# colmap/pycolmap

Hardware: AMD Instinct MI355X
Metric: descriptor-pair distances/sec (exhaustive SIFT match: dot + top-2 + ratio + cross-check) (higher is better)
Workload: dtype u8 descriptors, int8 MFMA / int32 accumulate; 1 GPU; 500 images x 4096 descriptors, exhaustive match + ratio test + cross-check (BASELINE.json configs[1] at N=1); pairs_total=124750, pairs_per_rank=124750, kernel=auto, matches_rank0=1865611

## Files before the change

### pycolmap_amd/csrc/match_mfma.hip

```cpp
#include <cstdlib>

#include "amc_internal.h"
#include "scan_accept.h"

namespace amc {

typedef int i32x4 __attribute__((ext_vector_type(4)));
typedef __attribute__((address_space(1))) const void gvoid_t;
typedef __attribute__((address_space(3))) void lvoid_t;

constexpr int kBN = 256;
constexpr int kYS = kBN / 32;
constexpr int kUR = 128;
constexpr int kSPB = kUR / 32;
constexpr int kUPC = kBN / kUR;
constexpr int kChunkBytes = kBN * kDim;
constexpr int kW = kSegsPerItem;
constexpr int kXT = kSegRows / 16;
constexpr int kKeyShift = 7, kKeyCarried = 127;

constexpr int kNB = 3;
constexpr int kOffRs = 0;
constexpr int kOffQ = kOffRs + kNB * kBN * 4;
constexpr int kOffB = kOffQ + 16;
constexpr int kLdsBytes = kOffB + kNB * kChunkBytes;
static_assert(kBN == kRowPad, "a chunk is the row padding unit");
static_assert(kUR == 128 && kSPB == 4, "a lane quarter's rows of a block are one 32-row tile; the loop body is one block");
static_assert(kRowPad % kSegRows == 0 && kSegRows % 32 == 0, "segments tile the padded rows");
static_assert(kLdsBytes <= 160 * 1024, "LDS of one CU");
static_assert(sizeof(SegDesc) == 64, "a descriptor is 16 dwords: one per lane of a quarter wave");

enum : int { kDXprep = 0, kDXrs = 2, kDOut = 4, kDList = 6, kDYprep = 8, kDYrs = 10, kDCnt = 12, kDAccword = 13,
             kDYrows = 14 };

__device__ __forceinline__ void mfma_first(i32x4& d, const i32x4& a, const i32x4& b, const i32x4& c) {
    asm volatile("v_mfma_i32_16x16x64_i8 %0, %1, %2, %3" : "=&v"(d) : "v"(a), "v"(b), "v"(c));
}
__device__ __forceinline__ void mfma_acc(i32x4& d, const i32x4& a, const i32x4& b) {
    asm volatile("v_mfma_i32_16x16x64_i8 %0, %1, %2, %0" : "+v"(d) : "v"(a), "v"(b));
}

struct YFrag {
    i32x4 f[2][2];
    i32x4 ci[2];
};

#ifdef AMC_SCAN_STAMPS
constexpr int kStampMaxWG = 1024;
__device__ uint32_t g_scan_stamps[2 * kStampMaxWG * kSegsPerItem * 8];
#define AMC_STAMP() ((uint32_t)__builtin_amdgcn_s_memtime())
#endif

__device__ __noinline__ __attribute__((used)) void copy_part(const uint4* __restrict__ src, uint4* __restrict__ dst,
                                                             unsigned long long b, unsigned long long e, int tid,
                                                             int nthreads) {
    __builtin_assume(tid >= 0 && tid < 1024 && nthreads >= 256 && nthreads <= 512);
    unsigned long long i = b + (unsigned long long)tid;
    const unsigned long long st = (unsigned long long)nthreads;
    for (; i + 3 * st < e; i += 4 * st) {
        const uint4 v0 = src[i], v1 = src[i + st], v2 = src[i + 2 * st], v3 = src[i + 3 * st];
        dst[i] = v0; dst[i + st] = v1; dst[i + 2 * st] = v2; dst[i + 3 * st] = v3;
    }
    for (; i < e; i += st) dst[i] = src[i];
}

template <int MODE>
__global__ __launch_bounds__(64 * kW) void match_mfma_kernel(const SegDesc* __restrict__ segs,
                                                             const uint32_t* __restrict__ nitems_p,
                                                             uint32_t* __restrict__ queue_head,
                                                             uint32_t* __restrict__ accmask,
                                                             const ScanAccept* __restrict__ accept,
                                                             CopyJob job, uint32_t* __restrict__ copy_head) {
    static_assert((kChunkBytes / 1024) % kW == 0 && kYS % (kChunkBytes / 1024 / kW) == 0, "a chunk splits into 1 KiB DMA pieces per wave, dealt evenly over its steps");
    __shared__ __attribute__((aligned(16))) char smem[kLdsBytes];

    const int tid = threadIdx.x;
    const int lane = tid & 63;
    const int wid = __builtin_amdgcn_readfirstlane(tid >> 6);
    const int l15 = lane & 15, lq = lane >> 4;
    volatile uint32_t* s_q = reinterpret_cast<volatile uint32_t*>(smem + kOffQ);
    if constexpr (MODE == 0) {
        if (job.parts) {
            __shared__ uint32_t s_part;
            if (tid == 0) s_part = atomicAdd(copy_head, 1u);
            __syncthreads();
            const uint32_t part = s_part;
            if (part < job.parts)
                copy_part(static_cast<const uint4*>(job.src), static_cast<uint4*>(job.dst), job.n16 * part / job.parts,
                          job.n16 * (part + 1) / job.parts, tid, 64 * kW);
        }
    }
    const uint32_t nitems = *nitems_p;
    const ScanAccept sa = *accept;

    auto load_desc = [&](uint32_t q) -> int {
        int v = 0;
        if (q < nitems && lane < 16) v = reinterpret_cast<const int*>(segs + (size_t)q * kSegsPerItem + wid)[lane];
        return v;
    };
    auto dword = [&](int dv, int f) -> int { return __builtin_amdgcn_readlane(dv, f); };
    auto dptr = [&](int dv, int f) -> const char* {
        const uint64_t lo = (uint32_t)__builtin_amdgcn_readlane(dv, f);
        const uint64_t hi = (uint32_t)__builtin_amdgcn_readlane(dv, f + 1);
        return reinterpret_cast<const char*>(lo | (hi << 32));
    };

    constexpr int kPW = kChunkBytes / 1024 / kW;
    auto stage_piece = [&](const char* yprep, int c, int buf, int ps) __attribute__((always_inline)) {
        const int piece = ps * kW + wid;
        __builtin_amdgcn_global_load_lds((gvoid_t*)(yprep + (size_t)c * kChunkBytes + piece * 1024 + lane * 16),
                                         (lvoid_t*)(smem + kOffB + buf * kChunkBytes + piece * 1024), 16, 0, 0);
    };
    auto stage_rs = [&](const char* yrs, int c, int buf) __attribute__((always_inline)) {
        if (wid == 0)
            __builtin_amdgcn_global_load_lds((gvoid_t*)(yrs + (size_t)c * kBN * 4 + lane * 16),
                                             (lvoid_t*)(smem + kOffRs + buf * kBN * 4), 16, 0, 0);
    };
    auto stage = [&](const char* yprep, const char* yrs, int c, int buf) __attribute__((always_inline)) {
#pragma unroll
        for (int ps = 0; ps < kPW; ++ps) stage_piece(yprep, c, buf, ps);
        stage_rs(yrs, c, buf);
    };

    const int yrow_lane = (kUR / 4) * (l15 >> 2) + (l15 & 3);
    const int ysw_lane = arena_swizzle(yrow_lane);
    const int yoff0 = kOffB + yrow_lane * kDim + ((lq ^ ysw_lane) * 16);
    const int yoff1 = kOffB + yrow_lane * kDim + (((4 + lq) ^ ysw_lane) * 16);
    const int coff = kOffRs + (kUR / 4) * lq * 4;
    auto load_y_part = [&](YFrag& y, int buf, int ys, int part) __attribute__((always_inline)) {
        const int ub = (ys / kSPB) * kUR, sp = ys % kSPB;
        if (part < 2) {
            const int so = buf * kBN * 4 + (ub + 8 * sp) * 4;
            y.ci[part] = *reinterpret_cast<const i32x4*>(smem + (coff + so) + 16 * part);
        } else {
            const int tt = (part - 2) >> 1, s = (part - 2) & 1;
            const int so = buf * kChunkBytes + (ub + 8 * sp) * kDim;
            y.f[tt][s] = *reinterpret_cast<const i32x4*>(smem + ((s ? yoff1 : yoff0) + so) + tt * 4 * kDim);
        }
    };
    auto load_y = [&](YFrag& y, int buf, int ys) __attribute__((always_inline)) {
#pragma unroll
        for (int part = 0; part < 6; ++part) load_y_part(y, buf, ys, part);
    };

    i32x4 xf[kXT][2];
    int best[kXT], sec[kXT], btile[kXT], xterm[kXT], part[kXT];
    auto load_x = [&](int dv) __attribute__((always_inline)) {
        const int cnt = dword(dv, kDCnt);
        const char* xprep = dptr(dv, kDXprep);
        const int* xrs = reinterpret_cast<const int*>(dptr(dv, kDXrs));
#pragma unroll
        for (int xt = 0; xt < kXT; ++xt) {
            const int kl = xt * 16 + l15;
            int row;
            if (MODE == 0) {
                row = kl;
            } else {
                const uint32_t* list = reinterpret_cast<const uint32_t*>(dptr(dv, kDList));
                row = cnt > 0 ? (int)list[min(kl, cnt - 1)] : 0;
            }
            const char* rp = xprep + (size_t)row * kDim;
            const int sw = arena_swizzle(row);
#pragma unroll
            for (int s = 0; s < 2; ++s) xf[xt][s] = *reinterpret_cast<const i32x4*>(rp + (((4 * s + lq) ^ sw) * 16));
            xterm[xt] = xrs[row] - (1 << 21);
            best[xt] = ((-xterm[xt]) << kKeyShift) | kKeyCarried;
            sec[xt] = best[xt];
            btile[xt] = -1;
        }
    };

#ifdef AMC_SCAN_STAMPS
    uint32_t st_a = 0, st_first = 0, st_end = 0, st_sum[5] = {0, 0, 0, 0, 0};
    bool st_prev = false, st_prev_active = false;
    uint32_t* const st_slot = g_scan_stamps + ((size_t)(MODE * kStampMaxWG + min((int)blockIdx.x, kStampMaxWG - 1)) * kW + wid) * 8;
#endif
    if (tid == 0) *s_q = atomicAdd(queue_head, 1u);
    __syncthreads();
    uint32_t q = *s_q;
    int dv = load_desc(q);
    if (q < nitems) {
        stage(dptr(dv, kDYprep), dptr(dv, kDYrs), 0, 0);
        if (dword(dv, kDYrows) > kBN) stage(dptr(dv, kDYprep), dptr(dv, kDYrs), 1, 1);
        if (dword(dv, kDCnt) > 0) load_x(dv);
    }
    __syncthreads();

    while (q < nitems) {
        const char* yprep = dptr(dv, kDYprep);
        const char* yrs = dptr(dv, kDYrs);
        const int yrows_item = dword(dv, kDYrows);
        const int nchunks = (yrows_item + kBN - 1) / kBN;
        const int last_steps = (((yrows_item - (nchunks - 1) * kBN) + 31) / 32 + kSPB - 1) & ~(kSPB - 1);
        const bool active = dword(dv, kDCnt) > 0;
        if (tid == 0) *s_q = atomicAdd(queue_head, 1u);

        i32x4 acc[2][2];
        auto insert = [&](int xt, int code) __attribute__((always_inline)) {
            asm volatile(
                "v_lshl_or_b32 %2, %2, 7, %3\n\t"
                "v_med3_i32 %1, %0, %1, %2\n\t"
                "v_max_i32 %0, %0, %2"
                : "+v"(best[xt]), "+v"(sec[xt]), "+v"(part[xt])
                : "s"(code));
        };
        auto flush = [&](int sb) __attribute__((always_inline)) {
#pragma unroll
            for (int xt = 0; xt < kXT; ++xt) {
                const int c = best[xt] & 127;
                btile[xt] = c != kKeyCarried ? sb * 64 + (126 - c) : btile[xt];
                best[xt] |= kKeyCarried;
            }
        };
        auto phase = [&](i32x4 (&an)[2], const YFrag& y, int xtn, const i32x4 (&ac)[2], int xtc, int sp, int gb)
                         __attribute__((always_inline)) {
            mfma_first(an[0], y.f[0][0], xf[xtn][0], y.ci[0]);
            mfma_first(an[1], y.f[1][0], xf[xtn][0], y.ci[1]);
            __builtin_amdgcn_sched_barrier(0);
            if (xtc == 0 ? sp == 0 : sp == kSPB - 1) {
                insert((xtc + kXT - 1) % kXT, 126 - ((xtc == 0 ? gb - 1 : gb) & 63));
                if (xtc == 0 && gb != 0 && (gb & 63) == 0) flush((gb >> 6) - 1);
                __builtin_amdgcn_sched_barrier(0);
            }
            mfma_acc(an[0], y.f[0][1], xf[xtn][1]);
            mfma_acc(an[1], y.f[1][1], xf[xtn][1]);
            __builtin_amdgcn_sched_barrier(0);
            int t0, t1;
            if (sp == 0)
                asm volatile(
                    "v_max3_i32 %0, %3, %4, %5\n\t"
                    "v_max3_i32 %1, %6, %7, %8\n\t"
                    "v_max3_i32 %0, %0, %9, %10\n\t"
                    "v_max_i32 %2, %0, %1"
                    : "=&v"(t0), "=&v"(t1), "=&v"(part[xtc])
                    : "v"(ac[0][0]), "v"(ac[0][1]), "v"(ac[0][2]), "v"(ac[0][3]), "v"(ac[1][0]), "v"(ac[1][1]),
                      "v"(ac[1][2]), "v"(ac[1][3]));
            else
                asm volatile(
                    "v_max3_i32 %0, %3, %4, %5\n\t"
                    "v_max3_i32 %1, %6, %7, %8\n\t"
                    "v_max3_i32 %0, %0, %9, %10\n\t"
                    "v_max3_i32 %2, %0, %1, %2"
                    : "=&v"(t0), "=&v"(t1), "+v"(part[xtc])
                    : "v"(ac[0][0]), "v"(ac[0][1]), "v"(ac[0][2]), "v"(ac[0][3]), "v"(ac[1][0]), "v"(ac[1][1]),
                      "v"(ac[1][2]), "v"(ac[1][3]));
            __builtin_amdgcn_sched_barrier(0);
        };

        YFrag y0, y1;
        asm volatile("s_waitcnt vmcnt(0)" ::: "memory");
        __syncthreads();
        const uint32_t qn = *s_q;
        const int dvn = load_desc(qn);
#ifdef AMC_SCAN_STAMPS
        {
            const uint32_t now = AMC_STAMP();
            if (st_prev) {
                st_sum[0] += st_a;
                st_sum[1] += now - st_end;
                st_sum[2] += now - st_first;
                st_sum[3] += 1;
                st_sum[4] += st_prev_active ? 1 : 0;
                if (lane == 0) {
#pragma unroll
                    for (int k = 0; k < 5; ++k) st_slot[k] = st_sum[k];
                }
            }
            st_a = 0;
            st_first = now;
        }
#endif
        if (active) {
            load_y(y0, 0, 0);
            mfma_first(acc[0][0], y0.f[0][0], xf[0][0], y0.ci[0]);
            mfma_first(acc[0][1], y0.f[1][0], xf[0][0], y0.ci[1]);
            mfma_acc(acc[0][0], y0.f[0][1], xf[0][1]);
            mfma_acc(acc[0][1], y0.f[1][1], xf[0][1]);
            part[kXT - 1] = -(1 << 24);
            __builtin_amdgcn_sched_barrier(0);
        }
        auto step = [&](YFrag& yc, YFrag& yn, int c, int cb, int nb, int ys, int sp) __attribute__((always_inline)) {
            const bool lastt = sp == kSPB - 1 && ys == kYS - 1;
            const bool cross = lastt && (c + 1 < nchunks);
            const bool fetch = c + 2 < nchunks;
            if (fetch) {
                const int fb = cb == 0 ? 2 : cb - 1;
                constexpr int kEvery = kYS / kPW;
                static_assert(kEvery == 2, "a DMA piece behind every other step");
                if (sp % kEvery == 0) stage_piece(yprep, c + 2, fb, ys / kEvery);
                if (ys == 0) stage_rs(yrs, c + 2, fb);
            }
            if (cross) {
#ifdef AMC_SCAN_STAMPS
                const uint32_t st_t = AMC_STAMP();
#endif
                if (!fetch) asm volatile("s_waitcnt vmcnt(0)" ::: "memory");
                else if (wid == 0) asm volatile("s_waitcnt vmcnt(%0)" ::"n"(kPW + 1) : "memory");
                else asm volatile("s_waitcnt vmcnt(%0)" ::"n"(kPW) : "memory");
                asm volatile("s_barrier" ::: "memory");
#ifdef AMC_SCAN_STAMPS
                st_a += AMC_STAMP() - st_t;
#endif
            }
            if (active) {
                const int nbuf = cross ? nb : cb;
                const int nys = lastt ? (cross ? 0 : ys) : ys + 1;
                const int gb = c * kUPC + ys / kSPB;
#pragma unroll
                for (int xt = 0; xt < kXT; ++xt) {
                    if (xt + 1 < kXT)
                        phase(acc[(xt + 1) & 1], yc, xt + 1, acc[xt & 1], xt, sp, gb);
                    else
                        phase(acc[0], yn, 0, acc[xt & 1], xt, sp, gb);
                    if (xt < 6) {
                        load_y_part(yn, nbuf, nys, xt);
                        __builtin_amdgcn_sched_barrier(0);
                    }
                }
            }
        };
        for (int c = 0, cb = 0; c < nchunks; ++c) {
            const int nb = cb == 2 ? 0 : cb + 1;
            const int yend = (c == nchunks - 1) ? last_steps : kYS;
#pragma unroll 1
            for (int ys = 0; ys < yend; ys += kSPB) {
                step(y0, y1, c, cb, nb, ys, 0);
                step(y1, y0, c, cb, nb, ys + 1, 1);
                step(y0, y1, c, cb, nb, ys + 2, 2);
                step(y1, y0, c, cb, nb, ys + 3, 3);
            }
            cb = nb;
        }
        if (active) {
            const int lastb = (nchunks - 1) * kUPC + last_steps / kSPB - 1;
            insert(kXT - 1, 126 - (lastb & 63));
            flush(lastb >> 6);
#pragma unroll
            for (int xt = 0; xt < kXT; ++xt) {
                best[xt] >>= kKeyShift;
                sec[xt] >>= kKeyShift;
            }
        }
        __syncthreads();
#ifdef AMC_SCAN_STAMPS
        st_end = AMC_STAMP();
        st_prev = true;
        st_prev_active = active;
#endif

        int eb[kXT], es[kXT], et[kXT], ex[kXT];
#pragma unroll
        for (int xt = 0; xt < kXT; ++xt) {
            asm volatile("v_mov_b32 %0, %1" : "=v"(eb[xt]) : "v"(best[xt]));
            asm volatile("v_mov_b32 %0, %1" : "=v"(es[xt]) : "v"(sec[xt]));
            asm volatile("v_mov_b32 %0, %1" : "=v"(et[xt]) : "v"(btile[xt]));
            ex[xt] = xterm[xt];
        }
        if (qn < nitems) {
            stage(dptr(dvn, kDYprep), dptr(dvn, kDYrs), 0, 0);
            if (dword(dvn, kDYrows) > kBN) stage(dptr(dvn, kDYprep), dptr(dvn, kDYrs), 1, 1);
            if (dword(dvn, kDCnt) > 0) load_x(dvn);
        }
        if (active) {
            const int cnt = dword(dv, kDCnt);
            uint32_t bits_lo = 0;
#pragma unroll
            for (int xt = 0; xt < kXT; ++xt) {
                const int kl = xt * 16 + l15;
                int b = eb[xt], s = es[xt], t = et[xt] < 0 ? -1 : et[xt] * kSPB + lq;
#pragma unroll
                for (int m = 16; m <= 32; m <<= 1) {
                    const int ob = __shfl_xor(b, m);
                    const int os = __shfl_xor(s, m);
                    const int ot = __shfl_xor(t, m);
                    const bool ow = (ob > b) || (ob == b && (unsigned)ot < (unsigned)t);
                    s = max(max(s, os), ow ? b : ob);
                    t = ow ? ot : t;
                    b = ow ? ob : b;
                }
                bool acc_bit = false;
                if (lq == 0 && kl < cnt) {
                    Top2* out = reinterpret_cast<Top2*>(const_cast<char*>(dptr(dv, kDOut)));
                    int row = kl;
                    if (MODE == 1) row = (int)reinterpret_cast<const uint32_t*>(dptr(dv, kDList))[kl];
                    Top2 o;
                    o.best_v = (uint32_t)(b + ex[xt]);
                    o.best_idx = o.best_v ? (uint32_t)t : 0xFFFFFFFFu;
                    o.second_v = (uint32_t)(s + ex[xt]);
                    o.pad = 0;
                    out[row] = o;
                    if (MODE == 0) acc_bit = scan_may_accept(sa, o.best_v, o.second_v);
                }
                if (MODE == 0) {
                    const uint32_t bits = (uint32_t)__ballot(acc_bit);
                    if (xt & 1) {
                        if (lane == 0) accmask[(uint32_t)dword(dv, kDAccword) + (xt >> 1)] = bits_lo | (bits << 16);
                    } else {
                        bits_lo = bits;
                    }
                }
            }
        }
#ifdef AMC_SCAN_STAMPS
        if (qn >= nitems && lane == 0) {
            st_slot[5] = st_a;
            st_slot[6] = AMC_STAMP() - st_first;
            st_slot[7] = 1;
        }
#endif
        q = qn;
        dv = dvn;
    }
}

__device__ __forceinline__ uint32_t pair_segments(int mode, const ImageDev* imgs, const PairDev& p, uint32_t pi,
                                                  const uint32_t* cand_cnt, uint32_t* nrows_out) {
    const uint32_t nx = mode == 0 ? imgs[p.slot1].rows : cand_cnt[pi];
    const uint32_t ny = imgs[mode == 0 ? p.slot2 : p.slot1].rows;
    *nrows_out = nx;
    return ny ? (nx + kSegRows - 1) / kSegRows : 0u;
}

__global__ __launch_bounds__(256) void seg_count_kernel(int mode, const ImageDev* __restrict__ imgs,
                                                        const PairDev* __restrict__ pairs,
                                                        const uint32_t* __restrict__ order,
                                                        const uint32_t* __restrict__ grp_start,
                                                        const uint32_t* __restrict__ cand_cnt,
                                                        uint32_t* __restrict__ seg_base, uint32_t* __restrict__ grp_segs) {
    __shared__ uint32_t wsum[4];
    const uint32_t g = blockIdx.x, tid = threadIdx.x, lane = tid & 63, wid = tid >> 6;
    const uint32_t i0 = grp_start[g], i1 = grp_start[g + 1];
    uint32_t running = 0;
    for (uint32_t base = i0; base < i1; base += 256) {
        const uint32_t i = base + tid;
        uint32_t s = 0, nr;
        if (i < i1) {
            const uint32_t pi = order[i];
            s = pair_segments(mode, imgs, pairs[pi], pi, cand_cnt, &nr);
        }
        uint32_t inc = s;
#pragma unroll
        for (int m = 1; m < 64; m <<= 1) {
            const uint32_t o = __shfl_up(inc, m);
            if (lane >= (uint32_t)m) inc += o;
        }
        if (lane == 63) wsum[wid] = inc;
        __syncthreads();
        uint32_t wbase = 0, total = 0;
        for (uint32_t k = 0; k < 4; ++k) {
            if (k < wid) wbase += wsum[k];
            total += wsum[k];
        }
        if (i < i1) seg_base[i] = running + wbase + inc - s;
        running += total;
        __syncthreads();
    }
    if (tid == 0) grp_segs[g] = running;
}

__global__ __launch_bounds__(1024) void seg_scan_kernel(const uint32_t* __restrict__ grp_segs, uint32_t ngroups,
                                                        uint32_t* __restrict__ grp_item_base,
                                                        uint32_t* __restrict__ nitems_out) {
    __shared__ uint32_t wsum[16];
    const uint32_t tid = threadIdx.x, lane = tid & 63, wid = tid >> 6;
    uint32_t running = 0;
    for (uint32_t base = 0; base < ngroups; base += 1024) {
        const uint32_t g = base + tid;
        const uint32_t s = g < ngroups ? (grp_segs[g] + kSegsPerItem - 1) / kSegsPerItem : 0u;
        uint32_t inc = s;
#pragma unroll
        for (int m = 1; m < 64; m <<= 1) {
            const uint32_t o = __shfl_up(inc, m);
            if (lane >= (uint32_t)m) inc += o;
        }
        if (lane == 63) wsum[wid] = inc;
        __syncthreads();
        uint32_t wbase = 0, total = 0;
        for (uint32_t k = 0; k < 16; ++k) {
            if (k < wid) wbase += wsum[k];
            total += wsum[k];
        }
        if (g < ngroups) grp_item_base[g] = running + wbase + inc - s;
        running += total;
        __syncthreads();
    }
    if (tid == 0) *nitems_out = running;
}

constexpr uint32_t kFillY = 8;
__global__ __launch_bounds__(256) void seg_fill_kernel(int mode, const ImageDev* __restrict__ imgs,
                                                       const PairDev* __restrict__ pairs,
                                                       const uint32_t* __restrict__ order,
                                                       const uint32_t* __restrict__ grp_start,
                                                       const uint32_t* __restrict__ cand_cnt,
                                                       const uint32_t* __restrict__ candbuf,
                                                       const uint32_t* __restrict__ seg_base,
                                                       const uint32_t* __restrict__ grp_segs,
                                                       const uint32_t* __restrict__ grp_item_base,
                                                       Top2* __restrict__ outbuf, SegDesc* __restrict__ segs) {
    const uint32_t g = blockIdx.x, tid = threadIdx.x, lane = tid & 63, wid = blockIdx.y * 4 + (tid >> 6);
    const uint32_t i0 = grp_start[g], i1 = grp_start[g + 1];
    if (i0 >= i1) return;
    const uint32_t total = grp_segs[g];
    if (total == 0) return;
    SegDesc* gs = segs + (size_t)grp_item_base[g] * kSegsPerItem;
    const PairDev p0 = pairs[order[i0]];
    const ImageDev Y = imgs[mode == 0 ? p0.slot2 : p0.slot1];
    for (uint32_t i = i0 + wid; i < i1; i += 4 * kFillY) {
        const uint32_t pi = order[i];
        const PairDev p = pairs[pi];
        uint32_t nx;
        const uint32_t ns = pair_segments(mode, imgs, p, pi, cand_cnt, &nx);
        const ImageDev X = imgs[mode == 0 ? p.slot1 : p.slot2];
        const uint32_t sb = seg_base[i];
        for (uint32_t k = lane; k < ns; k += 64) {
            const uint32_t row0 = k * kSegRows;
            SegDesc d;
            d.yprep = Y.prep;
            d.yrs = Y.rs128;
            d.yrows = Y.rows;
            d.cnt = min(nx - row0, (uint32_t)kSegRows);
            d.pad_ = 0;
            if (mode == 0) {
                d.xprep = X.prep + (size_t)row0 * kDim;
                d.xrs = X.rs128 + row0;
                d.out = outbuf + p.row_off + row0;
                d.list = nullptr;
                d.accword = (uint32_t)((p.row_off + row0) >> 5);
            } else {
                d.xprep = X.prep;
                d.xrs = X.rs128;
                d.out = outbuf + p.col_off;
                d.list = candbuf + p.col_off + row0;
                d.accword = 0;
            }
            gs[sb + k] = d;
        }
    }
    const uint32_t padded = (total + kSegsPerItem - 1) / kSegsPerItem * kSegsPerItem;
    if (blockIdx.y == 0 && tid < padded - total) {
        SegDesc d;
        d.xprep = Y.prep;
        d.xrs = Y.rs128;
        d.out = nullptr;
        d.list = nullptr;
        d.yprep = Y.prep;
        d.yrs = Y.rs128;
        d.cnt = 0;
        d.accword = 0;
        d.yrows = Y.rows;
        d.pad_ = 0;
        gs[total + tid] = d;
    }
}

hipError_t launch_build_segments(int mode, const ImageDev* imgs, const PairDev* pairs, const uint32_t* order,
                                 const uint32_t* grp_start, uint32_t ngroups, const uint32_t* cand_cnt,
                                 const uint32_t* candbuf, Top2* outbuf, uint32_t* seg_base, uint32_t* grp_segs,
                                 uint32_t* grp_item_base, SegDesc* segs, uint32_t* nitems_dev, hipStream_t s) {
    if (ngroups == 0) return memset_async(nitems_dev, 0, sizeof(uint32_t), s);
    hipLaunchKernelGGL(seg_count_kernel, dim3(ngroups), dim3(256), 0, s, mode, imgs, pairs, order, grp_start,
                       cand_cnt, seg_base, grp_segs);
    hipLaunchKernelGGL(seg_scan_kernel, dim3(1), dim3(1024), 0, s, grp_segs, ngroups, grp_item_base, nitems_dev);
    hipLaunchKernelGGL(seg_fill_kernel, dim3(ngroups, kFillY), dim3(256), 0, s, mode, imgs, pairs, order, grp_start,
                       cand_cnt, candbuf, seg_base, grp_segs, grp_item_base, outbuf, segs);
    return hipGetLastError();
}

hipError_t launch_match_mfma(int mode, const SegDesc* segs, const uint32_t* nitems_dev, uint32_t max_items,
                             uint32_t* queue_head, uint32_t* accmask, const ScanAccept* accept_dev, hipStream_t s,
                             const CopyJob& job_in, uint32_t* copy_head) {
    if (max_items == 0) return hipSuccess;
    CopyJob job = (mode == 0 && copy_head) ? job_in : CopyJob();
    hipError_t e = job.parts ? memset_async(copy_head, 0, sizeof(uint32_t), s) : hipSuccess;
    if (e != hipSuccess) return e;
    int dev = 0, cus = 256;
    if ((e = hipGetDevice(&dev)) != hipSuccess) return e;
    if ((e = hipDeviceGetAttribute(&cus, hipDeviceAttributeMultiprocessorCount, dev)) != hipSuccess) return e;
    static const int grid_cap = [] {
        const char* e = std::getenv("AMC_SCAN_GRID");
        return e ? std::atoi(e) : 0;
    }();
    if (grid_cap > 0 && grid_cap < cus) cus = grid_cap;
    const uint32_t grid = max_items < (uint32_t)cus ? max_items : (uint32_t)cus;
    if (job.parts > grid) job.parts = grid;
    if ((e = memset_async(queue_head, 0, sizeof(uint32_t), s)) != hipSuccess) return e;
    if (mode == 0)
        hipLaunchKernelGGL((match_mfma_kernel<0>), dim3(grid), dim3(64 * kW), 0, s, segs, nitems_dev, queue_head,
                           accmask, accept_dev, job, copy_head);
    else
        hipLaunchKernelGGL((match_mfma_kernel<1>), dim3(grid), dim3(64 * kW), 0, s, segs, nitems_dev, queue_head,
                           accmask, accept_dev, job, copy_head);
    return hipGetLastError();
}

}
```

Before: 13450 billion distances/s.

## Stream Y chunks across work items with a 4-deep ring and lookahead queue

```diff
diff --git a/pycolmap_amd/csrc/match_mfma.hip b/pycolmap_amd/csrc/match_mfma.hip
--- a/pycolmap_amd/csrc/match_mfma.hip
+++ b/pycolmap_amd/csrc/match_mfma.hip
@@ -2,12 +2,15 @@
 
 #include "amc_internal.h"
 #include "scan_accept.h"
+#include "scan_schedule.h"
 
 namespace amc {
 
 typedef int i32x4 __attribute__((ext_vector_type(4)));
 typedef __attribute__((address_space(1))) const void gvoid_t;
 typedef __attribute__((address_space(3))) void lvoid_t;
+typedef __attribute__((address_space(3))) volatile uint32_t lds_u32_t;
+template <typename T> using gptr_t = __attribute__((address_space(1))) T*;
 
 constexpr int kBN = 256;
 constexpr int kYS = kBN / 32;
@@ -19,12 +22,12 @@
 constexpr int kXT = kSegRows / 16;
 constexpr int kKeyShift = 7, kKeyCarried = 127;
 
-constexpr int kNB = 3;
+constexpr int kNB = sched::kRing;
 constexpr int kOffRs = 0;
 constexpr int kOffQ = kOffRs + kNB * kBN * 4;
-constexpr int kOffB = kOffQ + 16;
+constexpr int kOffB = kOffQ + 4 * sched::kQueueRing;
 constexpr int kLdsBytes = kOffB + kNB * kChunkBytes;
-static_assert(kBN == kRowPad, "a chunk is the row padding unit");
+static_assert(kBN == kRowPad && kBN == sched::kChunkRows && kUR == sched::kHalfRows && kNB == 4, "scan_schedule.h describes this stream");
 static_assert(kUR == 128 && kSPB == 4, "a lane quarter's rows of a block are one 32-row tile; the loop body is one block");
 static_assert(kRowPad % kSegRows == 0 && kSegRows % 32 == 0, "segments tile the padded rows");
 static_assert(kLdsBytes <= 160 * 1024, "LDS of one CU");
@@ -78,7 +81,7 @@
     const int lane = tid & 63;
     const int wid = __builtin_amdgcn_readfirstlane(tid >> 6);
     const int l15 = lane & 15, lq = lane >> 4;
-    volatile uint32_t* s_q = reinterpret_cast<volatile uint32_t*>(smem + kOffQ);
+    lds_u32_t* const s_q = (lds_u32_t*)(smem + kOffQ);
     if constexpr (MODE == 0) {
         if (job.parts) {
             __shared__ uint32_t s_part;
@@ -157,13 +160,19 @@
                 row = kl;
             } else {
                 const uint32_t* list = reinterpret_cast<const uint32_t*>(dptr(dv, kDList));
-                row = cnt > 0 ? (int)list[min(kl, cnt - 1)] : 0;
+                row = cnt > 0 ? (int)*(gptr_t<const uint32_t>)(list + min(kl, cnt - 1)) : 0;
             }
             const char* rp = xprep + (size_t)row * kDim;
             const int sw = arena_swizzle(row);
 #pragma unroll
-            for (int s = 0; s < 2; ++s) xf[xt][s] = *reinterpret_cast<const i32x4*>(rp + (((4 * s + lq) ^ sw) * 16));
-            xterm[xt] = xrs[row] - (1 << 21);
+            for (int s = 0; s < 2; ++s) xf[xt][s] = *(gptr_t<const i32x4>)(rp + (((4 * s + lq) ^ sw) * 16));
+            xterm[xt] = *(gptr_t<const int>)(xrs + row);
+        }
+    };
+    auto init_x = [&]() __attribute__((always_inline)) {
+#pragma unroll
+        for (int xt = 0; xt < kXT; ++xt) {
+            xterm[xt] -= 1 << 21;
             best[xt] = ((-xterm[xt]) << kKeyShift) | kKeyCarried;
             sec[xt] = best[xt];
             btile[xt] = -1;
@@ -172,140 +181,164 @@
 
 #ifdef AMC_SCAN_STAMPS
     uint32_t st_a = 0, st_first = 0, st_end = 0, st_sum[5] = {0, 0, 0, 0, 0};
-    bool st_prev = false, st_prev_active = false;
     uint32_t* const st_slot = g_scan_stamps + ((size_t)(MODE * kStampMaxWG + min((int)blockIdx.x, kStampMaxWG - 1)) * kW + wid) * 8;
 #endif
-    if (tid == 0) *s_q = atomicAdd(queue_head, 1u);
+    if (tid < sched::kQueueAhead) s_q[tid] = atomicAdd(queue_head, 1u);
     __syncthreads();
-    uint32_t q = *s_q;
-    int dv = load_desc(q);
-    if (q < nitems) {
-        stage(dptr(dv, kDYprep), dptr(dv, kDYrs), 0, 0);
-        if (dword(dv, kDYrows) > kBN) stage(dptr(dv, kDYprep), dptr(dv, kDYrs), 1, 1);
-        if (dword(dv, kDCnt) > 0) load_x(dv);
-    }
+    auto load_descs = [&](uint32_t j0, bool last_only) -> int {
+        int v = 0;
+        if (!last_only || lq == sched::kDescAhead) {
+            const uint32_t id = s_q[sched::queue_slot(j0 + (uint32_t)lq)];
+            int dw = l15;
+            asm volatile("" : "+v"(dw));
+            if (id < nitems) v = reinterpret_cast<const int*>(segs + (size_t)id * kSegsPerItem + wid)[dw];
+        }
+        return v;
+    };
+    struct YInfo {
+        const char* yprep;
+        const char* yrs;
+        int nchunks;
+    };
+    auto yinfo = [&](int d, int k) -> YInfo {
+        YInfo y;
+        const uint64_t plo = (uint32_t)__builtin_amdgcn_readlane(d, 16 * k + kDYprep);
+        const uint64_t phi = (uint32_t)__builtin_amdgcn_readlane(d, 16 * k + kDYprep + 1);
+        const uint64_t rlo = (uint32_t)__builtin_amdgcn_readlane(d, 16 * k + kDYrs);
+        const uint64_t rhi = (uint32_t)__builtin_amdgcn_readlane(d, 16 * k + kDYrs + 1);
+        y.yprep = reinterpret_cast<const char*>(plo | (phi << 32));
+        y.yrs = reinterpret_cast<const char*>(rlo | (rhi << 32));
+        y.nchunks = sched::chunks_of(__builtin_amdgcn_readlane(d, 16 * k + kDYrows));
+        return y;
+    };
+    uint32_t js = 0;
+    int dq = load_descs(0, false);
+    YInfo F = yinfo(dq, 0);
+    sched::FetchPos fpos{0, 0u, 0u};
+    int pi = 0;
+    auto fetch_next = [&]() __attribute__((always_inline)) {
+        if (sched::fetch_advance(fpos, F.nchunks)) F = yinfo(dq, (int)(fpos.j - js));
+    };
+    auto issue_piece = [&]() __attribute__((always_inline)) {
+        if (F.nchunks != 0 && pi < kPW) {
+            const int fb = sched::ring_buf(fpos.v);
+            if (pi == 0) stage_rs(F.yrs, fpos.c, fb);
+            stage_piece(F.yprep, fpos.c, fb, pi);
+            ++pi;
+        }
+    };
+    auto pass_barrier = [&]() __attribute__((always_inline)) {
+        const bool fetching = F.nchunks != 0;
+        while (fetching && pi < kPW) issue_piece();
+#ifdef AMC_SCAN_STAMPS
+        const uint32_t st_t = AMC_STAMP();
+#endif
+        if (!fetching) asm volatile("s_waitcnt vmcnt(0)" ::: "memory");
+        else if (wid == 0) asm volatile("s_waitcnt vmcnt(%0)" ::"n"(kPW + 1) : "memory");
+        else asm volatile("s_waitcnt vmcnt(%0)" ::"n"(kPW) : "memory");
+        asm volatile("s_barrier" ::: "memory");
+#ifdef AMC_SCAN_STAMPS
+        st_a += AMC_STAMP() - st_t;
+#endif
+        fetch_next();
+        pi = 0;
+    };
+
+    for (int k = 0; k < sched::kFetchAhead; ++k) {
+        if (F.nchunks != 0) stage(F.yprep, F.yrs, fpos.c, sched::ring_buf(fpos.v));
+        fetch_next();
+    }
+    bool active = dword(dq, kDCnt) > 0;
+    if (active) load_x(dq);
+    asm volatile("s_waitcnt vmcnt(0)" ::: "memory");
+    if (active) init_x();
     __syncthreads();
-
-    while (q < nitems) {
-        const char* yprep = dptr(dv, kDYprep);
-        const char* yrs = dptr(dv, kDYrs);
-        const int yrows_item = dword(dv, kDYrows);
-        const int nchunks = (yrows_item + kBN - 1) / kBN;
-        const int last_steps = (((yrows_item - (nchunks - 1) * kBN) + 31) / 32 + kSPB - 1) & ~(kSPB - 1);
-        const bool active = dword(dv, kDCnt) > 0;
-        if (tid == 0) *s_q = atomicAdd(queue_head, 1u);
-
-        i32x4 acc[2][2];
-        auto insert = [&](int xt, int code) __attribute__((always_inline)) {
+    if (dword(dq, kDYrows) == 0) return;
+
+    i32x4 acc[2][2];
+    auto insert = [&](int xt, int code) __attribute__((always_inline)) {
+        asm volatile(
+            "v_lshl_or_b32 %2, %2, 7, %3\n\t"
+            "v_med3_i32 %1, %0, %1, %2\n\t"
+            "v_max_i32 %0, %0, %2"
+            : "+v"(best[xt]), "+v"(sec[xt]), "+v"(part[xt])
+            : "s"(code));
+    };
+    auto flush = [&](int sb) __attribute__((always_inline)) {
+#pragma unroll
+        for (int xt = 0; xt < kXT; ++xt) {
+            const int c = best[xt] & 127;
+            btile[xt] = c != kKeyCarried ? sb * 64 + (126 - c) : btile[xt];
+            best[xt] |= kKeyCarried;
+        }
+    };
+    auto phase = [&](i32x4 (&an)[2], const YFrag& y, int xtn, const i32x4 (&ac)[2], int xtc, int sp, int gb)
+                     __attribute__((always_inline)) {
+        mfma_first(an[0], y.f[0][0], xf[xtn][0], y.ci[0]);
+        mfma_first(an[1], y.f[1][0], xf[xtn][0], y.ci[1]);
+        __builtin_amdgcn_sched_barrier(0);
+        if (xtc == 0 ? sp == 0 : sp == kSPB - 1) {
+            insert((xtc + kXT - 1) % kXT, 126 - ((xtc == 0 ? gb - 1 : gb) & 63));
+            if (xtc == 0 && gb != 0 && (gb & 63) == 0) flush((gb >> 6) - 1);
+            __builtin_amdgcn_sched_barrier(0);
+        }
+        mfma_acc(an[0], y.f[0][1], xf[xtn][1]);
+        mfma_acc(an[1], y.f[1][1], xf[xtn][1]);
+        __builtin_amdgcn_sched_barrier(0);
+        int t0, t1;
+        if (sp == 0)
             asm volatile(
-                "v_lshl_or_b32 %2, %2, 7, %3\n\t"
-                "v_med3_i32 %1, %0, %1, %2\n\t"
-                "v_max_i32 %0, %0, %2"
-                : "+v"(best[xt]), "+v"(sec[xt]), "+v"(part[xt])
-                : "s"(code));
-        };
-        auto flush = [&](int sb) __attribute__((always_inline)) {
-#pragma unroll
-            for (int xt = 0; xt < kXT; ++xt) {
-                const int c = best[xt] & 127;
-                btile[xt] = c != kKeyCarried ? sb * 64 + (126 - c) : btile[xt];
-                best[xt] |= kKeyCarried;
-            }
-        };
-        auto phase = [&](i32x4 (&an)[2], const YFrag& y, int xtn, const i32x4 (&ac)[2], int xtc, int sp, int gb)
-                         __attribute__((always_inline)) {
-            mfma_first(an[0], y.f[0][0], xf[xtn][0], y.ci[0]);
-            mfma_first(an[1], y.f[1][0], xf[xtn][0], y.ci[1]);
-            __builtin_amdgcn_sched_barrier(0);
-            if (xtc == 0 ? sp == 0 : sp == kSPB - 1) {
-                insert((xtc + kXT - 1) % kXT, 126 - ((xtc == 0 ? gb - 1 : gb) & 63));
-                if (xtc == 0 && gb != 0 && (gb & 63) == 0) flush((gb >> 6) - 1);
-                __builtin_amdgcn_sched_barrier(0);
-            }
-            mfma_acc(an[0], y.f[0][1], xf[xtn][1]);
-            mfma_acc(an[1], y.f[1][1], xf[xtn][1]);
-            __builtin_amdgcn_sched_barrier(0);
-            int t0, t1;
-            if (sp == 0)
-                asm volatile(
-                    "v_max3_i32 %0, %3, %4, %5\n\t"
-                    "v_max3_i32 %1, %6, %7, %8\n\t"
-                    "v_max3_i32 %0, %0, %9, %10\n\t"
-                    "v_max_i32 %2, %0, %1"
-                    : "=&v"(t0), "=&v"(t1), "=&v"(part[xtc])
-                    : "v"(ac[0][0]), "v"(ac[0][1]), "v"(ac[0][2]), "v"(ac[0][3]), "v"(ac[1][0]), "v"(ac[1][1]),
-                      "v"(ac[1][2]), "v"(ac[1][3]));
-            else
-                asm volatile(
-                    "v_max3_i32 %0, %3, %4, %5\n\t"
-                    "v_max3_i32 %1, %6, %7, %8\n\t"
-                    "v_max3_i32 %0, %0, %9, %10\n\t"
-                    "v_max3_i32 %2, %0, %1, %2"
-                    : "=&v"(t0), "=&v"(t1), "+v"(part[xtc])
-                    : "v"(ac[0][0]), "v"(ac[0][1]), "v"(ac[0][2]), "v"(ac[0][3]), "v"(ac[1][0]), "v"(ac[1][1]),
-                      "v"(ac[1][2]), "v"(ac[1][3]));
-            __builtin_amdgcn_sched_barrier(0);
-        };
-
-        YFrag y0, y1;
-        asm volatile("s_waitcnt vmcnt(0)" ::: "memory");
-        __syncthreads();
-        const uint32_t qn = *s_q;
-        const int dvn = load_desc(qn);
-#ifdef AMC_SCAN_STAMPS
-        {
-            const uint32_t now = AMC_STAMP();
-            if (st_prev) {
-                st_sum[0] += st_a;
-                st_sum[1] += now - st_end;
-                st_sum[2] += now - st_first;
-                st_sum[3] += 1;
-                st_sum[4] += st_prev_active ? 1 : 0;
-                if (lane == 0) {
-#pragma unroll
-                    for (int k = 0; k < 5; ++k) st_slot[k] = st_sum[k];
-                }
-            }
-            st_a = 0;
-            st_first = now;
-        }
-#endif
-        if (active) {
-            load_y(y0, 0, 0);
-            mfma_first(acc[0][0], y0.f[0][0], xf[0][0], y0.ci[0]);
-            mfma_first(acc[0][1], y0.f[1][0], xf[0][0], y0.ci[1]);
-            mfma_acc(acc[0][0], y0.f[0][1], xf[0][1]);
-            mfma_acc(acc[0][1], y0.f[1][1], xf[0][1]);
-            part[kXT - 1] = -(1 << 24);
-            __builtin_amdgcn_sched_barrier(0);
-        }
-        auto step = [&](YFrag& yc, YFrag& yn, int c, int cb, int nb, int ys, int sp) __attribute__((always_inline)) {
-            const bool lastt = sp == kSPB - 1 && ys == kYS - 1;
-            const bool cross = lastt && (c + 1 < nchunks);
-            const bool fetch = c + 2 < nchunks;
-            if (fetch) {
-                const int fb = cb == 0 ? 2 : cb - 1;
-                constexpr int kEvery = kYS / kPW;
-                static_assert(kEvery == 2, "a DMA piece behind every other step");
-                if (sp % kEvery == 0) stage_piece(yprep, c + 2, fb, ys / kEvery);
-                if (ys == 0) stage_rs(yrs, c + 2, fb);
-            }
-            if (cross) {
-#ifdef AMC_SCAN_STAMPS
-                const uint32_t st_t = AMC_STAMP();
-#endif
-                if (!fetch) asm volatile("s_waitcnt vmcnt(0)" ::: "memory");
-                else if (wid == 0) asm volatile("s_waitcnt vmcnt(%0)" ::"n"(kPW + 1) : "memory");
-                else asm volatile("s_waitcnt vmcnt(%0)" ::"n"(kPW) : "memory");
-                asm volatile("s_barrier" ::: "memory");
-#ifdef AMC_SCAN_STAMPS
-                st_a += AMC_STAMP() - st_t;
-#endif
-            }
+                "v_max3_i32 %0, %3, %4, %5\n\t"
+                "v_max3_i32 %1, %6, %7, %8\n\t"
+                "v_max3_i32 %0, %0, %9, %10\n\t"
+                "v_max_i32 %2, %0, %1"
+                : "=&v"(t0), "=&v"(t1), "=&v"(part[xtc])
+                : "v"(ac[0][0]), "v"(ac[0][1]), "v"(ac[0][2]), "v"(ac[0][3]), "v"(ac[1][0]), "v"(ac[1][1]),
+                  "v"(ac[1][2]), "v"(ac[1][3]));
+        else
+            asm volatile(
+                "v_max3_i32 %0, %3, %4, %5\n\t"
+                "v_max3_i32 %1, %6, %7, %8\n\t"
+                "v_max3_i32 %0, %0, %9, %10\n\t"
+                "v_max3_i32 %2, %0, %1, %2"
+                : "=&v"(t0), "=&v"(t1), "+v"(part[xtc])
+                : "v"(ac[0][0]), "v"(ac[0][1]), "v"(ac[0][2]), "v"(ac[0][3]), "v"(ac[1][0]), "v"(ac[1][1]),
+                  "v"(ac[1][2]), "v"(ac[1][3]));
+        __builtin_amdgcn_sched_barrier(0);
+    };
+
+    YFrag y0, y1;
+    const bool trail = sched::is_trail(wid);
+    sched::ScanPos pos{0, 0, 0u};
+    int nchunks = sched::chunks_of(dword(dq, kDYrows));
+    int last_halves = sched::last_halves_of(dword(dq, kDYrows));
+    auto prime = [&]() __attribute__((always_inline)) {
+        load_y(y0, sched::ring_buf(pos.v), 0);
+        mfma_first(acc[0][0], y0.f[0][0], xf[0][0], y0.ci[0]);
+        mfma_first(acc[0][1], y0.f[1][0], xf[0][0], y0.ci[1]);
+        mfma_acc(acc[0][0], y0.f[0][1], xf[0][1]);
+        mfma_acc(acc[0][1], y0.f[1][1], xf[0][1]);
+        part[kXT - 1] = -(1 << 24);
+        __builtin_amdgcn_sched_barrier(0);
+    };
+    if (active) prime();
+#ifdef AMC_SCAN_STAMPS
+    st_first = AMC_STAMP();
+#endif
+#pragma unroll 1
+    for (;;) {
+        const sched::HalfPlan pl = sched::plan_half(pos, nchunks, last_halves, trail);
+        const sched::ScanPos nx = sched::next_half(pos, pl);
+        const int cb = sched::ring_buf(pos.v), nb = sched::ring_buf(nx.v);
+        const int gb = pos.c * kUPC + pos.h;
+        auto step = [&](YFrag& yc, YFrag& yn, int sp) __attribute__((always_inline)) {
+            const bool lastt = sp == kSPB - 1;
+            const int ys = pos.h * kSPB + sp;
+            if (sched::piece_step(sp)) issue_piece();
+            if (lastt && pl.barrier) pass_barrier();
             if (active) {
-                const int nbuf = cross ? nb : cb;
-                const int nys = lastt ? (cross ? 0 : ys) : ys + 1;
-                const int gb = c * kUPC + ys / kSPB;
+                const int nbuf = lastt && !pl.item_ends ? nb : cb;
+                const int nys = lastt ? (pl.item_ends ? ys : nx.h * kSPB) : ys + 1;
 #pragma unroll
                 for (int xt = 0; xt < kXT; ++xt) {
                     if (xt + 1 < kXT)
@@ -319,35 +352,25 @@
                 }
             }
         };
-        for (int c = 0, cb = 0; c < nchunks; ++c) {
-            const int nb = cb == 2 ? 0 : cb + 1;
-            const int yend = (c == nchunks - 1) ? last_steps : kYS;
-#pragma unroll 1
-            for (int ys = 0; ys < yend; ys += kSPB) {
-                step(y0, y1, c, cb, nb, ys, 0);
-                step(y1, y0, c, cb, nb, ys + 1, 1);
-                step(y0, y1, c, cb, nb, ys + 2, 2);
-                step(y1, y0, c, cb, nb, ys + 3, 3);
-            }
-            cb = nb;
-        }
+        step(y0, y1, 0);
+        step(y1, y0, 1);
+        step(y0, y1, 2);
+        step(y1, y0, 3);
+        pos = nx;
+        if (!pl.item_ends) continue;
+
+#ifdef AMC_SCAN_STAMPS
+        st_end = AMC_STAMP();
+#endif
         if (active) {
-            const int lastb = (nchunks - 1) * kUPC + last_steps / kSPB - 1;
-            insert(kXT - 1, 126 - (lastb & 63));
-            flush(lastb >> 6);
+            insert(kXT - 1, 126 - (gb & 63));
+            flush(gb >> 6);
 #pragma unroll
             for (int xt = 0; xt < kXT; ++xt) {
                 best[xt] >>= kKeyShift;
                 sec[xt] >>= kKeyShift;
             }
         }
-        __syncthreads();
-#ifdef AMC_SCAN_STAMPS
-        st_end = AMC_STAMP();
-        st_prev = true;
-        st_prev_active = active;
-#endif
-
         int eb[kXT], es[kXT], et[kXT], ex[kXT];
 #pragma unroll
         for (int xt = 0; xt < kXT; ++xt) {
@@ -356,13 +379,21 @@
             asm volatile("v_mov_b32 %0, %1" : "=v"(et[xt]) : "v"(btile[xt]));
             ex[xt] = xterm[xt];
         }
-        if (qn < nitems) {
-            stage(dptr(dvn, kDYprep), dptr(dvn, kDYrs), 0, 0);
-            if (dword(dvn, kDYrows) > kBN) stage(dptr(dvn, kDYprep), dptr(dvn, kDYrs), 1, 1);
-            if (dword(dvn, kDCnt) > 0) load_x(dvn);
-        }
-        if (active) {
-            const int cnt = dword(dv, kDCnt);
+        const bool was_active = active;
+        const int cnt = dword(dq, kDCnt);
+        const uint32_t accword = (uint32_t)dword(dq, kDAccword);
+        Top2* const out = reinterpret_cast<Top2*>(const_cast<char*>(dptr(dq, kDOut)));
+        const uint32_t* const list = reinterpret_cast<const uint32_t*>(dptr(dq, kDList));
+        uint32_t popped = 0;
+        if (tid == 0)
+            asm volatile("global_atomic_add %0, %1, %2, %3 sc0" : "=&v"(popped) : "v"(0), "v"(1), "s"(queue_head) : "memory");
+        ++js;
+        const int dsh = __shfl(dq, (lane + 16) & 63);
+        const int dnew = load_descs(js, true);
+        const bool more = dword(dsh, kDYrows) != 0;
+        active = dword(dsh, kDCnt) > 0;
+        auto decode_store = [&]() __attribute__((always_inline)) {
+          if (was_active) {
             uint32_t bits_lo = 0;
 #pragma unroll
             for (int xt = 0; xt < kXT; ++xt) {
@@ -380,36 +411,66 @@
                 }
                 bool acc_bit = false;
                 if (lq == 0 && kl < cnt) {
-                    Top2* out = reinterpret_cast<Top2*>(const_cast<char*>(dptr(dv, kDOut)));
                     int row = kl;
-                    if (MODE == 1) row = (int)reinterpret_cast<const uint32_t*>(dptr(dv, kDList))[kl];
+                    if (MODE == 1) row = (int)*(gptr_t<const uint32_t>)(list + kl);
                     Top2 o;
                     o.best_v = (uint32_t)(b + ex[xt]);
                     o.best_idx = o.best_v ? (uint32_t)t : 0xFFFFFFFFu;
                     o.second_v = (uint32_t)(s + ex[xt]);
-                    o.pad = 0;
-                    out[row] = o;
+                                        const i32x4 ov = {(int)o.best_v, (int)o.best_idx, (int)o.second_v, 0};
+                    *(gptr_t<i32x4>)(out + row) = ov;
                     if (MODE == 0) acc_bit = scan_may_accept(sa, o.best_v, o.second_v);
                 }
                 if (MODE == 0) {
                     const uint32_t bits = (uint32_t)__ballot(acc_bit);
                     if (xt & 1) {
-                        if (lane == 0) accmask[(uint32_t)dword(dv, kDAccword) + (xt >> 1)] = bits_lo | (bits << 16);
+                        if (lane == 0) accmask[accword + (xt >> 1)] = bits_lo | (bits << 16);
                     } else {
                         bits_lo = bits;
                     }
                 }
             }
-        }
-#ifdef AMC_SCAN_STAMPS
-        if (qn >= nitems && lane == 0) {
-            st_slot[5] = st_a;
-            st_slot[6] = AMC_STAMP() - st_first;
-            st_slot[7] = 1;
-        }
-#endif
-        q = qn;
-        dv = dvn;
+          }
+        };
+        load_x(more ? dsh : dq);
+        decode_store();
+        dq = lq == sched::kDescAhead ? dnew : dsh;
+        asm volatile("s_waitcnt vmcnt(0)" ::: "memory");
+        asm volatile("" : "+v"(dq), "+v"(popped));
+        init_x();
+        if (tid == 0) {
+            s_q[sched::queue_slot(js + sched::kQueueAhead - 1)] = popped;
+            asm volatile("s_waitcnt lgkmcnt(0)" ::: "memory");
+        }
+        if (!more) {
+#ifdef AMC_SCAN_STAMPS
+            if (lane == 0) {
+                st_slot[5] = st_a;
+                st_slot[6] = AMC_STAMP() - st_first;
+                st_slot[7] = 1;
+            }
+#endif
+            break;
+        }
+        nchunks = sched::chunks_of(dword(dq, kDYrows));
+        last_halves = sched::last_halves_of(dword(dq, kDYrows));
+        if (active) prime();
+#ifdef AMC_SCAN_STAMPS
+        {
+            const uint32_t now = AMC_STAMP();
+            st_sum[0] += st_a;
+            st_sum[1] += now - st_end;
+            st_sum[2] += now - st_first;
+            st_sum[3] += 1;
+            st_sum[4] += was_active ? 1 : 0;
+            if (lane == 0) {
+#pragma unroll
+                for (int k = 0; k < 5; ++k) st_slot[k] = st_sum[k];
+            }
+            st_a = 0;
+            st_first = now;
+        }
+#endif
     }
 }
 
diff --git a/pycolmap_amd/csrc/scan_schedule.h b/pycolmap_amd/csrc/scan_schedule.h
--- /dev/null
+++ b/pycolmap_amd/csrc/scan_schedule.h
@@ -0,0 +1,73 @@
+#pragma once
+
+#if defined(__HIPCC__)
+#define AMC_SCHED_FN __host__ __device__ __forceinline__
+#else
+#define AMC_SCHED_FN inline
+#endif
+
+namespace amc {
+namespace sched {
+
+constexpr int kChunkRows = 256;
+constexpr int kHalfRows = 128;
+constexpr int kRing = 4;
+constexpr int kFetchAhead = 2;
+constexpr int kLeadWaves = 4;
+constexpr int kQueueRing = 8;
+constexpr int kQueueAhead = 5;
+constexpr int kDescAhead = 3;
+
+AMC_SCHED_FN int chunks_of(int yrows) { return (yrows + kChunkRows - 1) / kChunkRows; }
+AMC_SCHED_FN int last_halves_of(int yrows) {
+    return (yrows - (chunks_of(yrows) - 1) * kChunkRows + kHalfRows - 1) / kHalfRows;
+}
+AMC_SCHED_FN bool is_trail(int wave) { return wave >= kLeadWaves; }
+AMC_SCHED_FN int ring_buf(unsigned v) { return (int)(v % (unsigned)kRing); }
+AMC_SCHED_FN int queue_slot(unsigned j) { return (int)(j % (unsigned)kQueueRing); }
+
+struct ScanPos {
+    int c, h;
+    unsigned v;
+};
+struct HalfPlan {
+    bool leaves_chunk;
+    bool item_ends;
+    bool barrier;
+};
+AMC_SCHED_FN HalfPlan plan_half(const ScanPos& p, int nchunks, int last_halves, bool trail) {
+    HalfPlan pl;
+    const bool last_chunk = p.c == nchunks - 1;
+    pl.leaves_chunk = p.h == 1 || (last_chunk && last_halves < 2);
+    pl.item_ends = pl.leaves_chunk && last_chunk;
+    pl.barrier = trail ? p.h == 0 : pl.leaves_chunk;
+    return pl;
+}
+AMC_SCHED_FN ScanPos next_half(const ScanPos& p, const HalfPlan& pl) {
+    ScanPos n = p;
+    if (!pl.leaves_chunk) {
+        n.h = 1;
+    } else {
+        n.h = 0;
+        n.c = pl.item_ends ? 0 : p.c + 1;
+        n.v = p.v + 1;
+    }
+    return n;
+}
+
+struct FetchPos {
+    int c;
+    unsigned j, v;
+};
+AMC_SCHED_FN bool fetch_advance(FetchPos& f, int nchunks) {
+    if (nchunks == 0) return false;
+    ++f.v;
+    if (++f.c < nchunks) return false;
+    f.c = 0;
+    ++f.j;
+    return true;
+}
+AMC_SCHED_FN bool piece_step(int sp) { return (sp & 1) == 0; }
+
+}
+}
```

Result: slower. 13280 billion distances/s (-1.3%).
